# digitalcytometry/cytospace

Hardware: AMD Instinct MI355X
Metric: cell-to-spot assignments/sec on NxN synthetic cost; bit-exact vs lapjv (higher is better)
Workload: dtype f32

## Files before the change

cytospace_amd/csrc/lap_wide.hip:

```cpp
#include "lap_dev.h"
#include "lap_wide.h"
#include <algorithm>
#include <atomic>
#include <chrono>
#include <mutex>
#include <thread>
#include <vector>

namespace cyto {

#define WIDE_FIELDS(P, S)                                                                                                  \
    S(int, n) S(int64_t, ld) P(const float, cost) P(const int32_t, rowmap) P(float, v) P(float, u) P(float, cassign)          \
    P(unsigned long long, label) P(unsigned long long, bid) P(int32_t, rowsol) P(int32_t, colsol) P(int32_t, matches)          \
    P(int32_t, freerows) P(int32_t, act0) P(int32_t, act1) P(int32_t, touched) P(int32_t, slot_j) P(float, slot_p)            \
    P(float, slot_c) P(uint32_t, cache_col) P(float, cache_val) P(char, misc) S(long long, max_rounds)                     \
    P(const int32_t, same_prev) P(int32_t, seg_sync) S(int, aug_seg) S(int, aug_waste) S(int, arr_waste) S(int, seg_quorum)   \
    P(char, sc) S(int, par_groups) P(char, par) P(char, scx) P(float, cache_red) P(const int32_t, inv_off) P(const unsigned long long, inv_ent)
#define WIDE_F_PTR(T, name) T *name;
#define WIDE_F_VAL(T, name) T name;
struct WideArgs { WIDE_FIELDS(WIDE_F_PTR, WIDE_F_VAL) };

constexpr size_t WIDE_SC_BYTES = 2048;

namespace {
// ... 978 lines not shown
    int numfree = 0;
    for (int i0 = 0; i0 < n; i0 += WT) {
        const int i = i0 + tid;
        const bool fr = i < n && ld_sc1(a.rowsol + i) < 0;
        const uint64_t m = __ballot(fr);
        if (lane == 0) s.wcnt[w] = __popcll(m);
        __syncthreads();
        int pre = 0, tot = 0;
#pragma unroll
        for (int k = 0; k < WNW; k++) { const int c = s.wcnt[k]; if (k < w) pre += c; tot += c; }
        if (fr) a.freerows[numfree + pre + __popcll(m & lanemask_lt())] = i;
        numfree += tot;
        __syncthreads();
    }
    if (tid == 0) {
        long long *ctr = lap_status(a.misc)->counters;
        long long *wc = lap_status(a.misc)->wide;
        ctr[C_ARR] = bids; ctr[C_FREE_CR] = free_cr; ctr[C_FREE_A1] = numfree; ctr[C_FREE_A2] = numfree;
        wc[WC_ROUNDS] = round; wc[WC_BIDS] = bids; wc[WC_RETIRED] = s.retired; wc[WC_ACTIVE_LEFT] = left;
        wc[WC_FREE_ARR] = numfree; wc[WC_DENSE_ARR] = s.dense;
        lap_status(a.misc)->numfree = numfree;
        long long *tmr = lap_status(a.misc)->timers;
        tmr[WT_LIST_ROUNDS] = n_list; tmr[WT_LIST_TICKS] += t_list; tmr[WT_CHAIN_ROUNDS] = n_chain; tmr[WT_CHAIN_TICKS] += t_chain;
        tmr[WT_DEALS] = n_deal; tmr[WT_ARR_TAIL_TICKS] = wall_clock64() - t_tail0;
        h->started = 1; h->round = round; h->bids = bids; h->retired = s.retired; h->dense = s.dense; h->cnt[cur] = paused ? na : 0;
        h->cnt[cur ^ 1] = 0; h->free_cr = free_cr; h->done = paused ? 0 : 1; h->launches += 1; h->list_rounds = n_list;
#ifndef CYTO_WIDE_PROF
        tmr[WT_ARR_LAUNCHES] = h->launches;
#endif
        if (a.seg_sync) a.seg_sync[1 + blockIdx.x] = (paused ? 1 : 0) | ((!paused && s.dense <= n / 64) ? 2 : 0);
    }
}

struct ClaimCtl { int changed, blocked, rounds, pad_; };
__device__ __forceinline__ int *cl_claim(const WideArgs &a) { return reinterpret_cast<int *>(a.scx); }
__device__ __forceinline__ unsigned long long *cl_mask(const WideArgs &a) { return reinterpret_cast<unsigned long long *>(a.scx + sc_np(a.n) * 8); }
__device__ __forceinline__ int2 *cl_state(const WideArgs &a) { return reinterpret_cast<int2 *>(a.scx + sc_np(a.n) * 16); }
__device__ __forceinline__ ClaimCtl *cl_ctl(const WideArgs &a) { return reinterpret_cast<ClaimCtl *>(a.scx + sc_np(a.n) * 24); }
__device__ __forceinline__ int *cl_rem(const WideArgs &a) { return reinterpret_cast<int *>(a.scx + sc_np(a.n) * 32); }
constexpr int AP = 2;

size_t wide_aug_lds_bytes(int n, bool vlds, bool clds) {
    const size_t nblk = ((size_t)n + 63) / 64, nw32 = ((size_t)n + 31) / 32, npad = ((size_t)n + 3) & ~(size_t)3;
    return ((nblk * 8 + 3 * nw32 * 4 + npad * ((vlds ? 4 : 0) + (clds ? 2 : 0)) + 15) / 16) * 16;
}
bool wide_aug_vlds(int n) { return n <= 65534 && wide_aug_lds_bytes(n, true, true) + 4096 <= (size_t)LDS_DYNAMIC_MAX; }
bool wide_aug_clds(int n) { return n <= 65534 && wide_aug_lds_bytes(n, false, true) + 4096 <= (size_t)LDS_DYNAMIC_MAX; }

struct AugShared {
    unsigned long long T;
    int ntouch, any[3], npk[3], fail, anydense, rootdense, doroot, f, err;
    int waste, stop;
    int nhop;
    int conflict;
    int scans;
    int st_row[64], st_col[64];
    float st_val[64];
};
static_assert(WNW * AP <= 32, "the queue of a round's full-row relaxations: two halves of the 64-entry staging arrays");

struct ParCtl {
    unsigned int bar_arrive, bar_gen;
    int P[2], nplog[2], nolog[2];
    int err, pad_;
    long long c_relax, c_hops, c_proc, c_dense, c_rounds, c_verify, c_batches, c_discarded;
};
static_assert(sizeof(ParCtl) <= 256, "control block");
constexpr int PAR_GMAX = 64;
static size_t wide_par_state_bytes(int n, int G) {
    const size_t np = ((size_t)n + 63) & ~(size_t)63;
    return 256 + (size_t)G * np * 8 + (size_t)G * np * 4 + (size_t)G * np * 8 + np * 4 + np * 8 + np * 8;
}
__device__ __forceinline__ void par_barrier(ParCtl *c, int G, unsigned &gen) {
    __syncthreads();
    if (threadIdx.x == 0) {
        __builtin_amdgcn_fence(__ATOMIC_RELEASE, "agent");
        asm volatile("s_waitcnt vmcnt(0)" ::: "memory");
        const unsigned arrived = atomicAdd(&c->bar_arrive, 1u) + 1u;
        if (arrived == (gen + 1u) * (unsigned)G) st_sc1(&c->bar_gen, gen + 1u);
        else {
            long long spins = 0;
            while (ld_sc1(&c->bar_gen) <= gen) {
                __builtin_amdgcn_s_sleep(2);
                if (++spins > (1ll << 26)) { atomicExch(&c->err, 2); break; }
            }
        }
        __builtin_amdgcn_fence(__ATOMIC_ACQUIRE, "agent");
    }
    gen++;
    __syncthreads();
}

#ifndef CYTO_COOP_MIN_N
#define CYTO_COOP_MIN_N 16384
#endif
constexpr int COOP_MIN_N = CYTO_COOP_MIN_N;
template <bool VLDS>
__device__ __forceinline__ void coop_dense_rows(AugShared *sp, int nd, const float *__restrict__ cost, const int32_t *__restrict__ rowmap, int64_t ld,
                                             int n, int w, int lane, unsigned long long *lbl, int32_t *tch, uint32_t *dirty,
                                             unsigned long long *bmin, const uint32_t *asg, const float *s_v, const float *v) {
    AugShared &s = *sp;
    const int nq = (n + 3) >> 2, per = (nq + WNW - 1) / WNW, q_lo = w * per, q_hi = min(nq, q_lo + per);
    for (int e = 0; e < nd; e++) {
        const int oiq = uni(s.st_row[e]), pjq = uni(s.st_row[32 + e]);
        const uint32_t dord = (uint32_t)uni(s.st_col[e]), kq = (uint32_t)uni(s.st_col[32 + e]);
        const float h = uni(s.st_val[e]);
        const float *__restrict__ row = cost + wrow_off(rowmap, oiq, ld);
        wave_row_sweep_q(row, q_lo, q_hi, n, lane, [&](int c, float x) {
            const float vc = VLDS ? s_v[c] : ld_sc1(v + c);
            const unsigned long long lv = edge_lv(f2ord((x - vc) - h), dord, kq);
            const unsigned long long key = lkey(lv, (uint32_t)oiq);
            if (c == pjq || lv > lv_of(s.T) || !(key < ld_sc1(lbl + c))) return;
            const unsigned long long old = atomicMin(lbl + c, key);
            if (key < old) {
                if (old == ~0ull) tch[atomicAdd(&s.ntouch, 1)] = c;
                if (lv_of(old) > lv) {
                    const unsigned long long ck = lkey(lv, (uint32_t)c);
                    if ((asg[c >> 5] >> (c & 31)) & 1u) { atomicOr(&dirty[c >> 5], 1u << (c & 31)); atomicMin(&bmin[c >> 6], ck); }
                    else atomicMin(&s.T, ck);
                }
            }
        });
    }
    __syncthreads();
}

typedef __attribute__((address_space(1))) float gf32_t;
typedef __attribute__((address_space(1))) const int32_t gci32_t;
typedef __attribute__((address_space(1))) const unsigned long long gcu64_t;
__device__ __noinline__ void embed_repair(gf32_t *cache_red, gci32_t *inv_off, gcu64_t *inv_ent, uint64_t m, int k, float nv) {
    constexpr int U = 8;
    const int lane = threadIdx.x & 63;
    m = uni((unsigned long long)m);
    const bool mine = (m >> lane) & 1;
    const int e0 = mine ? inv_off[k] : 0, e1 = mine ? inv_off[k + 1] : 0;
    while (m) {
        int b[U], e[U]; float x[U]; unsigned long long t[U];
#pragma unroll
        for (int u = 0; u < U; u++) {
            const int l = m ? __ffsll((unsigned long long)m) - 1 : 0;
            b[u] = m ? __builtin_amdgcn_readlane(e0, l) : 0;
            e[u] = m ? __builtin_amdgcn_readlane(e1, l) : 0;
            x[u] = __uint_as_float((uint32_t)__builtin_amdgcn_readlane((int)__float_as_uint(nv), l));
            m &= m - 1;
        }
#pragma unroll
        for (int u = 0; u < U; u++) t[u] = b[u] + lane < e[u] ? inv_ent[b[u] + lane] : 0ull;
#pragma unroll
        for (int u = 0; u < U; u++) if (b[u] + lane < e[u]) cache_red[(uint32_t)t[u]] = __uint_as_float((uint32_t)(t[u] >> 32)) - x[u];
#pragma unroll
        for (int u = 0; u < U; u++)
            for (int p = b[u] + 64 + lane; p < e[u]; p += 64) { const unsigned long long y = inv_ent[p]; cache_red[(uint32_t)y] = __uint_as_float((uint32_t)(y >> 32)) - x[u]; }
    }
}

template <bool VLDS, bool CLDS, bool PAR, bool EMB = false>
__global__ __launch_bounds__(WT) void wide_aug(const WideArgs *__restrict__ batch) {
    static_assert(!EMB || (PAR && !VLDS), "the embedded form: several searches at once, prices in global memory");
    extern __shared__ __align__(16) unsigned char w_smem[];
    __shared__ AugShared s;
    const int pstride = PAR ? (int)(gridDim.x / (unsigned)load_wide_args(batch, 0).par_groups) : 1;
    if (PAR && (blockIdx.x % pstride)) return;
    const int g = PAR ? uni((int)(blockIdx.x / pstride)) : 0;
    const WideArgs a = load_wide_args(batch, PAR ? 0 : blockIdx.x);
    const int n = a.n, tid = threadIdx.x, lane = tid & 63, w = uni((int)(threadIdx.x >> 6));
    const int nblk = (n + 63) / 64, nw32 = (n + 31) / 32;
    const int G = PAR ? a.par_groups : 1;
    const size_t np_ = ((size_t)n + 63) & ~(size_t)63;
    ParCtl *pc = reinterpret_cast<ParCtl *>(a.par);
    unsigned long long *lbl = PAR ? reinterpret_cast<unsigned long long *>(a.par + 256) + (size_t)g * np_ : a.label;
    int32_t *tch = PAR ? reinterpret_cast<int32_t *>(a.par + 256 + (size_t)G * np_ * 8) + (size_t)g * np_ : a.touched;
    int32_t *hop_i = PAR ? reinterpret_cast<int32_t *>(a.par + 256 + (size_t)G * np_ * 12) + (size_t)g * 2 * np_ : a.act0;
    int32_t *hop_j = PAR ? hop_i + np_ : a.act1;
    uint32_t *claim = reinterpret_cast<uint32_t *>(a.par + 256 + (size_t)G * np_ * 20);
    int32_t *plog_col = reinterpret_cast<int32_t *>(claim + np_);
    float *plog_val = reinterpret_cast<float *>(plog_col + np_);
    int32_t *olog_col = reinterpret_cast<int32_t *>(plog_val + np_);
    int32_t *olog_own = olog_col + np_;
    unsigned pgen = 0;
    unsigned long long *bmin = reinterpret_cast<unsigned long long *>(w_smem);
    uint32_t *dirty = reinterpret_cast<uint32_t *>(bmin + nblk);
    uint32_t *asg = dirty + nw32;
    uint32_t *dense = asg + nw32;
    float *s_v = reinterpret_cast<float *>(dense + nw32);
    uint16_t *s_cs = reinterpret_cast<uint16_t *>(s_v + (VLDS ? ((n + 3) & ~3) : 0));
    const int numfree = lap_status(a.misc)->numfree;
    for (int b = tid; b < nblk; b += WT) bmin[b] = ~0ull;
    for (int q = tid; q < nw32; q += WT) { dirty[q] = 0; dense[q] = 0; }
    for (int c0 = 0; c0 < nw32 * 32; c0 += WT) {
        const int c = c0 + tid;
        const uint64_t m = __ballot(c < n && a.colsol[c] >= 0);
        if (lane == 0 && (c >> 5) < nw32) { asg[c >> 5] = (uint32_t)m; if ((c >> 5) + 1 < nw32) asg[(c >> 5) + 1] = (uint32_t)(m >> 32); }
    }
    if (CLDS)
        for (int j = tid; j < n; j += WT) {
            if (VLDS) s_v[j] = a.v[j];
            const int o = a.colsol[j]; s_cs[j] = o < 0 ? (uint16_t)0xFFFFu : (uint16_t)o;
        }
    const int f0 = PAR ? 0 : lap_status(a.misc)->wide_done;
    if (!PAR) {
        long long *wc = lap_status(a.misc)->wide;
        if (wc[WC_AUG_LAUNCHES] > 0 && f0 >= numfree) {
            if (tid == 0 && a.seg_sync) a.seg_sync[1 + blockIdx.x] = 0;
            return;
        }
    }
    if (tid == 0) { s.waste = 0; s.stop = 0; }
    if (tid == 0) { s.T = ~0ull; s.ntouch = 0; s.any[0] = 0; s.any[1] = 0; s.any[2] = 0; s.npk[0] = 0; s.npk[1] = 0; s.npk[2] = 0; s.fail = 0; s.anydense = 0; s.rootdense = 0; s.doroot = 0; s.f = f0; s.err = 0; s.scans = 0; }
    __syncthreads();
    auto getv = [&](int j) -> float { return VLDS ? s_v[j] : ld_sc1(a.v + j); };
    auto getcs = [&](int j) -> int {
        if (CLDS) { const uint16_t x = s_cs[j]; return x == 0xFFFFu ? -1 : (int)x; }
        return ld_sc1(a.colsol + j);
    };
    auto is_asg = [&](int c) -> bool { return (asg[c >> 5] >> (c & 31)) & 1u; };

    long long c_relax = 0, c_hops = 0, c_rounds = 0, c_proc = 0, c_trivial = 0, c_dense = 0, c_verify = 0;
    long long t_rounds = 0, t_verify = 0, t_finish = 0, t_triv = 0, t_mark = wall_clock64();

#define AUG_LAP(acc) { const long long now_ = wall_clock64(); acc += now_ - t_mark; t_mark = now_; }

    auto offer = [&](int col, unsigned long long lv, int row) -> unsigned long long {
        return atomicMin(lbl + col, lkey(lv, (uint32_t)row));
    };
    auto after_offer = [&](int col, unsigned long long lv, int row, unsigned long long old) {
        const unsigned long long key = lkey(lv, (uint32_t)row);
        if (key < old) {
            if (old == ~0ull) tch[atomicAdd(&s.ntouch, 1)] = col;
            if (lv_of(old) > lv) {
                const unsigned long long ck = lkey(lv, (uint32_t)col);
                if (is_asg(col)) { atomicOr(&dirty[col >> 5], 1u << (col & 31)); atomicMin(&bmin[col >> 6], ck); }
                else atomicMin(&s.T, ck);
            }
        }
    };
    auto relax_to = [&](int col, unsigned long long lv, int row) { after_offer(col, lv, row, offer(col, lv, row)); };

    int f = f0;
    int ph = 0;
    int rb[AP];
#pragma unroll
    for (int q = 0; q < AP; q++) rb[q] = -1;
    int seg_done = 0;
    int wact = 4;
    bool announced = false;
    int fbase = 0, batchno = 1, perr = 0;
    long long c_batches = 0, c_discarded = 0;
    for (;;) {
        if (!PAR && w == 0) {
            auto flush_one_edge = [&](int cnt) {
                if (lane < cnt) {
                    const int r = s.st_row[lane], cc = s.st_col[lane];
                    a.rowsol[r] = cc; a.colsol[cc] = r; a.cassign[cc] = s.st_val[lane];
                }
            };
            const int *remp = (a.same_prev && a.scx) ? cl_rem(a) : nullptr;
            int nst = 0;
            int p0, l0, r0, p1, l1, r1, p2, l2, r2, p3, l3v, r3v;
            uint32_t col0, col1, col2; float val0, val1, val2, vv0, vv1;
            auto start = [&](int ff) {
                auto len_of = [&](int pp) -> int { return pp < numfree ? (remp ? uni(remp[pp]) : 1) : 1; };
                auto row_at = [&](int pp) -> int { return pp < numfree ? uni(a.freerows[pp]) : -1; };
                p0 = ff; l0 = len_of(p0); r0 = row_at(p0);
                p1 = p0 + l0; l1 = len_of(p1); r1 = row_at(p1);
                p2 = p1 + l1; l2 = len_of(p2); r2 = row_at(p2);
                p3 = p2 + l2; l3v = p3 < numfree ? (remp ? remp[p3] : 1) : 1; r3v = p3 < numfree ? a.freerows[p3] : -1;
                col0 = COLSENT; col1 = COLSENT; col2 = COLSENT; val0 = 0.0f; val1 = 0.0f; val2 = 0.0f;
                if (r0 >= 0) { col0 = a.cache_col[(int64_t)r0 * KC + lane]; val0 = a.cache_val[(int64_t)r0 * KC + lane]; }
                if (r1 >= 0) { col1 = a.cache_col[(int64_t)r1 * KC + lane]; val1 = a.cache_val[(int64_t)r1 * KC + lane]; }
                if (r2 >= 0) { col2 = a.cache_col[(int64_t)r2 * KC + lane]; val2 = a.cache_val[(int64_t)r2 * KC + lane]; }
                vv0 = (r0 >= 0 && lane < KCU && col0 != COLSENT) ? getv((int)col0) : 0.0f;
                vv1 = (r1 >= 0 && lane < KCU && col1 != COLSENT) ? getv((int)col1) : 0.0f;
            };
// ... 227 lines not shown
                ph = (ph + 1) % 3;
                c_rounds++;
                wact = np > 6 ? WNW : 4;
                nd = npd >> 16;
                if (!any || nd) break;
            }
            if (nd) {
                coop_dense_rows<VLDS>(&s, nd, a.cost, a.rowmap, a.ld, n, w, lane, lbl, tch, dirty, bmin, asg, s_v, a.v);
                continue;
            }
            AUG_LAP(t_rounds)
            const unsigned long long Tk = s.T;
            const uint32_t Dord = (uint32_t)(Tk >> 32);
            const float D = Tk == ~0ull ? INFINITY : ord2f(Dord);
            const int nt = s.ntouch;
            for (int q = tid; q < nt; q += WT) {
                const int k = ld_sc1(tch + q);
                const unsigned long long lbk = ld_sc1(lbl + k);
                const uint32_t dord = (uint32_t)(lbk >> 32);
                if (lv_of(lbk) < lv_of(Tk) && is_asg(k)) {
                    const int i = getcs(k);
                    if (!((dense[i >> 5] >> (i & 31)) & 1u)) {
                        const float h = (ld_sc1(a.cassign + k) - getv(k)) - ord2f(dord);
                        const float bound = a.cache_val[(int64_t)i * KC + KCU] - h;
                        if (!(bound > D)) {
                            atomicOr(&dense[i >> 5], 1u << (i & 31));
                            atomicOr(&dirty[k >> 5], 1u << (k & 31));
                            atomicMin(&bmin[k >> 6], lkey(lv_of(lbk), (uint32_t)k));
                            atomicAdd(&s.fail, 1);
                        }
                    }
                }
            }
            if (tid == 0 && !s.rootdense && !(ftau > D)) { s.rootdense = 1; s.doroot = 1; atomicAdd(&s.fail, 1); }
            c_verify++;
            __syncthreads();
            const int fail = s.fail;
            if (s.doroot)
                for (int c = tid; c < n; c += WT) {
                    const unsigned long long lv = (unsigned long long)f2ord(frow[c] - getv(c)) << 12;
                    if (lv <= lv_of(s.T) && (lkey(lv, (uint32_t)fr) < ld_sc1(lbl + c))) relax_to(c, lv, fr);
                }
            __syncthreads();
            if (tid == 0) { if (fail) s.anydense = 1; s.fail = 0; s.doroot = 0; }
            __syncthreads();
            AUG_LAP(t_verify)
            if (!fail) break;
        }

        }

        const unsigned long long Tk = active ? s.T : ~0ull;
        if (!PAR && Tk == ~0ull) { if (tid == 0) s.err = 1; __syncthreads(); break; }
        const uint32_t Dord = (uint32_t)(Tk >> 32);
        const float D = ord2f(Dord);
        const int sink = (int)lid_of(Tk);
        const int nt = active ? s.ntouch : 0;
        bool commit = true;
        int Pb = G;
        const int par = batchno & 1;
        if (PAR) {
            const bool have = Tk != ~0ull;
            if (active && !have && tid == 0) atomicExch(&pc->err, 1);
            const uint32_t key = ((uint32_t)batchno << 8) | (uint32_t)(255 - g);
            if (have) {
                for (int q = tid; q < nt; q += WT) {
                    const int k = ld_sc1(tch + q);
                    if (lv_of(ld_sc1(lbl + k)) < lv_of(Tk) && is_asg(k)) atomicMax(claim + k, key);
                }
                if (tid == 0) atomicMax(claim + sink, key);
            }
            if (tid == 0) s.conflict = 0;
            par_barrier(pc, G, pgen);
            if (have) {
                int c = 0;
                for (int q = tid; q < nt; q += WT) {
                    const int k = ld_sc1(tch + q);
                    if (lv_of(ld_sc1(lbl + k)) < lv_of(Tk) && is_asg(k) && ld_sc1(claim + k) != key) c = 1;
                }
                if (tid == 0 && ld_sc1(claim + sink) != key) c = 1;
                if (c) s.conflict = 1;
            }
            __syncthreads();
            if (tid == 0 && active && (s.conflict || !have)) atomicMin(&pc->P[par], g);
            par_barrier(pc, G, pgen);
            Pb = uni(ld_sc1(&pc->P[par]));
            Pb = Pb < G ? Pb : G;
            if (g == 0 && tid == 0) { st_sc1(&pc->P[par ^ 1], PAR_GMAX + 1); st_sc1(&pc->nplog[par ^ 1], 0); st_sc1(&pc->nolog[par ^ 1], 0); }
            commit = active && have && g < Pb;
            if (active && !commit) c_discarded++;
        }
        if (commit) {
            int myscans = 0;
            for (int q = tid; q < nt; q += WT) {
                const int k = ld_sc1(tch + q);
                const uint32_t dord = (uint32_t)(ld_sc1(lbl + k) >> 32);
                if (dord < Dord && is_asg(k)) {
                    const float vk = getv(k);
                    const float nv = (vk + ord2f(dord)) - D;
                    if (nv < vk) {
                        a.v[k] = nv; if (VLDS) s_v[k] = nv;
                        if (PAR) { const int e = atomicAdd(&pc->nplog[par], 1); plog_col[e] = k; plog_val[e] = nv; }
                    }
                    myscans++;
                }
            }
            if (myscans) atomicAdd(&s.scans, myscans);
            if (tid == 0) {
                int j = sink, nh = 0;
                for (;;) {
                    const int i = (int)lid_of(ld_sc1(lbl + j));
                    const int jn = ld_sc1(a.rowsol + i);
                    a.colsol[j] = i; a.rowsol[i] = j;
                    st_sc1(hop_i + nh, (int32_t)i); st_sc1(hop_j + nh, (int32_t)j); nh++;
                    if (CLDS) s_cs[j] = (uint16_t)i;
                    c_hops++;
                    if (i == fr) break;
                    j = jn;
                }
                s.nhop = nh;
                atomicOr(&asg[sink >> 5], 1u << (sink & 31));
            }
            __syncthreads();
            for (int q = tid; q < s.nhop; q += WT) {
                const int i = ld_sc1(hop_i + q), j = ld_sc1(hop_j + q);
                a.cassign[j] = a.cost[wrow_off(a.rowmap, i, a.ld) + j];
                if (PAR) { const int e = atomicAdd(&pc->nolog[par], 1); olog_col[e] = j; olog_own[e] = i; }
            }
        }
        for (int q = tid; q < nt; q += WT) {
            const int k = ld_sc1(tch + q);
            lbl[k] = ~0ull;
            atomicAnd(&dirty[k >> 5], ~(1u << (k & 31)));
            bmin[k >> 6] = ~0ull;
        }
        if (s.anydense) for (int q = tid; q < nw32; q += WT) dense[q] = 0;
        __syncthreads();
        if (tid == 0) { if (commit) c_relax += s.scans; s.scans = 0; s.T = ~0ull; s.ntouch = 0; s.anydense = 0; s.rootdense = 0; s.f = f + 1; }
        f++;
        __syncthreads();
        if (PAR) {
            par_barrier(pc, G, pgen);
            perr = uni(ld_sc1(&pc->err));
            const int npl = uni(ld_sc1(&pc->nplog[par])), nol = uni(ld_sc1(&pc->nolog[par]));
            if (VLDS) for (int e = tid; e < npl; e += WT) s_v[ld_sc1(plog_col + e)] = ld_sc1(plog_val + e);
            for (int e = tid; e < nol; e += WT) {
                const int col = ld_sc1(olog_col + e);
                if (CLDS) s_cs[col] = (uint16_t)ld_sc1(olog_own + e);
                atomicOr(&asg[col >> 5], 1u << (col & 31));
            }
            __syncthreads();
            const int left = numfree - fbase;
            fbase += Pb < left ? Pb : left;
            if (Pb < 1) perr = 1;
            if (EMB) {
                for (int e0 = (g * WNW + w) * 8; e0 < npl; e0 += G * WNW * 8) {
                    const bool have_e = lane < 8 && e0 + lane < npl;
                    const int k = have_e ? ld_sc1(plog_col + e0 + lane) : 0;
                    const float nv = have_e ? ld_sc1(plog_val + e0 + lane) : 0.0f;
                    embed_repair((gf32_t *)a.cache_red, (gci32_t *)a.inv_off, (gcu64_t *)a.inv_ent, __ballot(have_e), k, nv);
                }
                par_barrier(pc, G, pgen);
            }
            batchno++; c_batches++;
        }
        AUG_LAP(t_finish)
    }

    __syncthreads();
    __shared__ double s_tot[WNW];
    __shared__ long long s_wc[WNW][4];
    if (lane == 0) { s_wc[w][0] = c_proc; s_wc[w][1] = c_dense; s_wc[w][2] = c_trivial; s_wc[w][3] = (w == 0) ? c_hops : 0; }
    __syncthreads();
    long long proc = 0, dn = 0, triv = 0, hops0 = 0;
    for (int k = 0; k < WNW; k++) { proc += s_wc[k][0]; dn += s_wc[k][1]; triv += s_wc[k][2]; hops0 += s_wc[k][3]; }
    if (PAR) {
        if (tid == 0) {
            atomicAdd(reinterpret_cast<unsigned long long *>(&pc->c_relax), (unsigned long long)c_relax);
            atomicAdd(reinterpret_cast<unsigned long long *>(&pc->c_hops), (unsigned long long)hops0);
            atomicAdd(reinterpret_cast<unsigned long long *>(&pc->c_proc), (unsigned long long)proc);
            atomicAdd(reinterpret_cast<unsigned long long *>(&pc->c_dense), (unsigned long long)dn);
            atomicAdd(reinterpret_cast<unsigned long long *>(&pc->c_discarded), (unsigned long long)c_discarded);
            if (g == 0) { pc->c_rounds = c_rounds; pc->c_verify = c_verify; pc->c_batches = c_batches; }
        }
        par_barrier(pc, G, pgen);
        if (g != 0) return;
        c_relax = (long long)ld_sc1(reinterpret_cast<unsigned long long *>(&pc->c_relax));
        hops0 = (long long)ld_sc1(reinterpret_cast<unsigned long long *>(&pc->c_hops));
        proc = (long long)ld_sc1(reinterpret_cast<unsigned long long *>(&pc->c_proc));
        dn = (long long)ld_sc1(reinterpret_cast<unsigned long long *>(&pc->c_dense));
        f = perr || ld_sc1(&pc->err) ? f : numfree;
    }
    double tot = 0.0;
    for (int i = tid; i < n; i += WT) {
        const int j = ld_sc1(a.rowsol + i);
        if (j >= 0) {
            const float cij = ld_sc1(a.cassign + j);
            a.u[i] = cij - ld_sc1(a.v + j);
            tot += (double)cij;
        }
    }
#pragma unroll
    for (int off = 32; off > 0; off >>= 1) tot += __shfl_xor(tot, off);
    if (lane == 0) s_tot[w] = tot;
    __syncthreads();
    if (tid == 0) {
        double t = 0.0;
        for (int k = 0; k < WNW; k++) t += s_tot[k];
        const bool err = s.err || (PAR && (perr || ld_sc1(&pc->err)));
        LapStatus *st = lap_status(a.misc);
        st->total = t;
        long long *ctr = st->counters, *wc = st->wide;
        ctr[C_AUG_INIT] = numfree; ctr[C_AUG_RELAX] += c_relax; ctr[C_AUGS] = numfree; ctr[C_HOPS] += hops0;
        wc[WC_DENSE_AUG] += dn; wc[WC_AUG_LAUNCHES] += 1; wc[WC_AUG_ROUNDS] += c_rounds; wc[WC_AUG_PROCESSED] += proc; wc[WC_TRIVIAL] += triv; wc[WC_VERIFY_PASSES] += c_verify;
        if (err) st->status = 1;
        st->wide_done = err ? numfree : f;
// ... 428 lines not shown
        const int xcd_cus = std::max(1, pl.cache.cus / 8);
        const bool dup_rows = n >= 2 && (long long)j.ngroups * 5 < (long long)n * 4;
        int parg = nl != 1 ? 0 : (pl.par > 0 ? pl.par : (pl.par < 0 || dup_rows || n < 2048 ? 0 : 16));
        parg = std::min(std::min(parg, WIDE_PAR_GMAX), xcd_cus);
        if (parg == 1) parg = 0;
        if (parg > 1) {
            if (g_par_busy[device_slot].exchange(1) != 0) parg = 0;
            else par_slot.p = &g_par_busy[device_slot];
        }
        const size_t parb = parg > 0 ? wide_par_state_bytes(n, parg) : 0;
        const size_t sc_off = ((2 * nT + 255) / 256) * 256;
        const size_t par_off = sc_off + WIDE_SC_BYTES;
        const size_t scx_off = ((par_off + parb + 255) / 256) * 256;
        bool vlds_k, clds_k;
        wide_aug_lds_choice(n, vlds_k, clds_k);
        const bool emb_cand = parg > 1 && !vlds_k && n <= (1 << 25) && embed_knob != 0;
        const size_t emb_off = ((scx_off + wide_sc_ext_bytes(n) + 255) / 256) * 256;
        if ((rc = j.state->alloc(emb_cand ? emb_off + wide_embed_bytes(n) : scx_off + wide_sc_ext_bytes(n), stream))) return rc;
        WideArgs &wa = h_wa[(size_t)k];
        wa.cache_red = nullptr; wa.inv_off = nullptr; wa.inv_ent = nullptr;
        if (emb_cand) {
            char *eb = j.state->as<char>() + emb_off;
            wa.cache_red = reinterpret_cast<float *>(eb);
            wa.inv_off = reinterpret_cast<int32_t *>(eb + emb_a256((size_t)n * KC * 4));
            wa.inv_ent = reinterpret_cast<unsigned long long *>(eb + emb_off_ent(n));
        }
        wa.n = n; wa.ld = j.ld; wa.cost = j.cost; wa.rowmap = j.rowmap;
        wa.v = j.fws; wa.u = j.fws + n; wa.cassign = j.fws + 3 * (int64_t)n;
        wa.label = reinterpret_cast<unsigned long long *>(j.fws + 4 * (int64_t)n);
        wa.rowsol = j.iws; wa.colsol = j.iws + n; wa.matches = j.iws + 2 * (int64_t)n; wa.freerows = j.iws + 3 * (int64_t)n;
        wa.act0 = j.iws + 4 * (int64_t)n; wa.act1 = j.iws + 5 * (int64_t)n; wa.touched = j.iws + 6 * (int64_t)n;
        wa.slot_j = j.iws + 7 * (int64_t)n;
        wa.bid = reinterpret_cast<unsigned long long *>(j.iws + 8 * (int64_t)n);
        wa.slot_p = j.state->as<float>(); wa.slot_c = wa.slot_p + n;
        wa.cache_col = j.cache_col; wa.cache_val = j.cache_val; wa.misc = j.misc;
        wa.max_rounds = pl.rounds;
        wa.aug_seg = pl.rebuild;
        wa.aug_waste = (int)std::min<long long>(1 << 30, std::max<long long>(16, (2000000ll + (long long)nl * n * n / 100) / n));
        wa.arr_waste = std::max(8, wa.aug_waste / 3);
        if (CYTO_KNOB("CYTO_ARR_WASTE").set) wa.arr_waste = std::max(1, CYTO_KNOB("CYTO_ARR_WASTE").value);
        wa.seg_quorum = nl > 1 ? std::max(1, nl / 4) : 0;
        wa.seg_sync = nullptr;
        wa.same_prev = j.same;
        wa.sc = j.state->as<char>() + sc_off;
        CYTO_HIP(hipMemsetAsync(wa.sc, 0, WIDE_SC_BYTES, stream));
        wa.scx = j.state->as<char>() + scx_off;
        CYTO_HIP(hipMemsetAsync(wa.scx, 0, wide_sc_ext_bytes(n), stream));
        CYTO_HIP(hipMemsetAsync(wa.scx, 0xFF, wide_sc_ones_bytes(n), stream));
        wa.par_groups = parg; wa.par = nullptr;
        if (parg > 0) {
            const size_t np_ = ((size_t)n + 63) & ~(size_t)63;
            wa.par = j.state->as<char>() + par_off;
            CYTO_HIP(hipMemsetAsync(wa.par, 0, 256, stream));
            const int p_init[2] = {WIDE_PAR_GMAX + 1, WIDE_PAR_GMAX + 1};
            CYTO_HIP(hipMemcpyAsync(wa.par + 8, p_init, sizeof p_init, hipMemcpyHostToDevice, stream));
            CYTO_HIP(hipMemsetAsync(wa.par + 256, 0xFF, (size_t)parg * np_ * 8, stream));
            CYTO_HIP(hipMemsetAsync(wa.par + 256 + (size_t)parg * np_ * 20, 0, np_ * 4, stream));
            CYTO_HIP(hipStreamSynchronize(stream));
        }
        CYTO_HIP(hipMemcpyAsync(wa.cassign, wa.v, nT, hipMemcpyDeviceToDevice, stream));
        CYTO_HIP(hipMemsetAsync(wa.label, 0xFF, 2 * nT, stream));
        CYTO_HIP(hipMemsetAsync(wa.bid, 0xFF, 2 * nT, stream));
    }
    DevBuf d_wa, d_sync;
    if ((rc = d_wa.alloc(sizeof(WideArgs) * nl, stream)) || (rc = d_sync.alloc(sizeof(int32_t) * ((size_t)nl + 1), stream))) return rc;
    for (WideArgs &wa : h_wa) wa.seg_sync = d_sync.as<int32_t>();
    CYTO_HIP(hipMemcpyAsync(d_wa.p, h_wa.data(), sizeof(WideArgs) * nl, hipMemcpyHostToDevice, stream));
    if ((rc = wide_launch_rt(d_wa.as<WideArgs>(), nl, n, stream))) return rc;
    std::vector<int32_t> h_sync((size_t)nl + 1, 1);
    std::vector<int32_t> caches_fresh((size_t)nl, 0);
    using BuildFn = decltype(build_caches_of);
    auto rebuild_tramp = +[](void *ctx, const int32_t *flags) -> int { return (*static_cast<BuildFn *>(ctx))(flags); };
    for (int pass = 0;; pass++) {
        if (pass && (rc = build_caches_of(h_sync.data() + 1))) return rc;
        CYTO_HIP(hipMemsetAsync(d_sync.p, 0, sizeof(int32_t), stream));
        if ((rc = wide_launch_arr(d_wa.as<WideArgs>(), nl, n, stream, pl.wipe, pass > 0, d_sync.as<int32_t>(), rebuild_tramp, &build_caches_of,
                                  nl == 1 ? &h_wa[0] : nullptr))) return rc;
        if (h_wa[0].aug_seg != 0) break;
        CYTO_HIP(hipMemcpyAsync(h_sync.data(), d_sync.p, sizeof(int32_t) * ((size_t)nl + 1), hipMemcpyDeviceToHost, stream));
        CYTO_HIP(hipStreamSynchronize(stream));
        bool done = true;
        for (int k = 0; k < nl; k++) { done = done && (h_sync[(size_t)k + 1] & 1) == 0; caches_fresh[(size_t)k] = (h_sync[(size_t)k + 1] & 2) != 0; h_sync[(size_t)k + 1] &= 1; }
        if (done) break;
    }
    const int parg = h_wa[0].par_groups;
    for (int pass = 0;; pass++) {
        if (pass == 0) {
            std::vector<int32_t> need((size_t)nl);
            for (int k = 0; k < nl; k++) need[(size_t)k] = caches_fresh[(size_t)k] ? 0 : 1;
            if ((rc = build_caches_of(need.data()))) return rc;
        } else if ((rc = build_caches_of(h_sync.data() + 1))) return rc;
        if (pass == 0) CYTO_HIP(hipEventRecord(ev_arr_done, stream));
        if (pass == 0 && parg == 0) {
            bool dup = false;
            for (int k = 0; k < nl; k++) dup = dup || h_wa[(size_t)k].same_prev != nullptr;
            if (dup && (rc = wide_launch_claims(d_wa.as<WideArgs>(), nl, n, stream, d_sync.as<int32_t>()))) return rc;
        }
        bool embed = false;
        if (parg > 0 && h_wa[0].cache_red) {
            if ((rc = wide_build_embedded(h_wa[0], n, stream))) return rc;
            embed = embed_knob >= 2;
            if (!embed) {
                int32_t longest = 0;
                CYTO_HIP(hipMemcpyAsync(&longest, emb_counts(h_wa[0], n) + n, sizeof longest, hipMemcpyDeviceToHost, stream));
                CYTO_HIP(hipStreamSynchronize(stream));
                embed = longest <= EMB_GATE;
            }
        }
        CYTO_HIP(hipMemsetAsync(d_sync.p, 0, sizeof(int32_t), stream));
        if ((rc = wide_launch_aug(d_wa.as<WideArgs>(), nl, n, stream, parg, embed))) return rc;
        if (embed) g_embedded_solves.fetch_add(1);
        if (parg > 0) { CYTO_HIP(hipStreamSynchronize(stream)); break; }
        CYTO_HIP(hipMemcpyAsync(h_sync.data(), d_sync.p, sizeof(int32_t) * ((size_t)nl + 1), hipMemcpyDeviceToHost, stream));
        CYTO_HIP(hipStreamSynchronize(stream));
        bool done = true;
        for (int k = 0; k < nl; k++) done = done && h_sync[(size_t)k + 1] == 0;
        if (done) break;
    }
    return CYTO_OK;
}

void wide_info(cyto_lap_info *info, const LapStatus &h) {
    const long long *wc = h.wide, *tm = h.timers;
    info->wide = 1;
    info->aug_handover = -1;
    info->wide_rounds = wc[WC_ROUNDS]; info->wide_retired = wc[WC_RETIRED]; info->wide_dense_arr = wc[WC_DENSE_ARR];
    info->wide_dense_aug = wc[WC_DENSE_AUG]; info->wide_aug_rounds = wc[WC_AUG_ROUNDS]; info->wide_aug_settled = wc[WC_AUG_PROCESSED];
    info->wide_trivial = wc[WC_TRIVIAL]; info->wide_verify_passes = wc[WC_VERIFY_PASSES]; info->wide_aug_launches = wc[WC_AUG_LAUNCHES];
    info->wide_list_rounds = tm[WT_LIST_ROUNDS]; info->wide_chain_rounds = tm[WT_CHAIN_ROUNDS];
    info->wide_ms_list = tm[WT_LIST_TICKS] * 1e-5; info->wide_ms_chain = tm[WT_CHAIN_TICKS] * 1e-5;
    info->wide_ms_aug_rounds = tm[WT_AUG_ROUNDS_TICKS] * 1e-5; info->wide_ms_aug_verify = tm[WT_AUG_VERIFY_TICKS] * 1e-5;
    info->wide_ms_aug_finish = tm[WT_AUG_FINISH_TICKS] * 1e-5; info->wide_ms_aug_trivial = tm[WT_AUG_TRIVIAL_TICKS] * 1e-5;
    info->wide_arr_launches = tm[WT_ARR_LAUNCHES]; info->wide_scaled = tm[WT_SCALED]; info->wide_phases = tm[WT_PHASES];
    info->wide_par_batches = tm[WT_PAR_BATCHES]; info->wide_par_discarded = tm[WT_PAR_DISCARDED];
}

}

extern "C" long long cyto_wide_embedded_solves(void) { return cyto::g_embedded_solves.load(); }
```

Before: 1.337 million.

## Restructure parallel augment finish: single-barrier claim, parallel price update, link-based path walk

Moves the end-of-search commit into a separate noinline routine. The claim phase now detects conflicts from the atomicMax return value instead of a second barrier-and-verify pass, which removes one grid-wide barrier per batch. Settled columns are logged into a per-group set list that a later batched price update reads. The augmenting-path walk runs in wave 0, using precomputed row links with 4-hop jumps, while the other waves update prices concurrently. Hop writes are batched, log appends use wave-aggregated atomics, and a host stream sync plus an H2D copy are dropped. The cost is extra global state and more complex, riskier conflict logic.

```diff
diff --git a/cytospace_amd/csrc/lap_wide.hip b/cytospace_amd/csrc/lap_wide.hip
--- a/cytospace_amd/csrc/lap_wide.hip
+++ b/cytospace_amd/csrc/lap_wide.hip
@@ -1054,7 +1054,7 @@
     int ntouch, any[3], npk[3], fail, anydense, rootdense, doroot, f, err;
     int waste, stop;
     int nhop;
-    int conflict;
+    int nset;
     int scans;
     int st_row[64], st_col[64];
     float st_val[64];
@@ -1069,10 +1069,48 @@
 };
 static_assert(sizeof(ParCtl) <= 256, "control block");
 constexpr int PAR_GMAX = 64;
+#ifdef CYTO_AUG_FIN_SPLIT
+constexpr int FS_MAXB = 2048, FS_G = 16, FS_NP = 14;
+enum { FS_CLAIM, FS_WAIT1, FS_CHECK, FS_WAIT2, FS_UPDATE, FS_WALK, FS_COST, FS_RESET, FS_WAIT3, FS_REPAIR, FS_NTOUCH, FS_SETTLED, FS_HOPS, FS_ARRIVE };
+__device__ long long g_fs[FS_MAXB][FS_G][FS_NP];
+#define FS_OK (PAR && batchno - 1 < FS_MAXB && g < FS_G)
+#define FS_BEGIN() { if (PAR && tid == 0) { fs_mark = wall_clock64(); if (FS_OK) g_fs[batchno - 1][g][FS_ARRIVE] = fs_mark; } }
+#define FS_LAP(part) { if (PAR) { __syncthreads(); if (tid == 0) { const long long fsn_ = wall_clock64(); if (FS_OK) g_fs[batchno - 1][g][part] = fsn_ - fs_mark; fs_mark = fsn_; } } }
+#define FS_SET(part, val) { if (tid == 0 && FS_OK) g_fs[batchno - 1][g][part] = (val); }
+#define FS_COUNT() atomicAdd(&s.st_col[63], 1)
+#else
+#define FS_BEGIN()
+#define FS_LAP(part)
+#define FS_SET(part, val)
+#define FS_COUNT()
+#endif
 static size_t wide_par_state_bytes(int n, int G) {
     const size_t np = ((size_t)n + 63) & ~(size_t)63;
-    return 256 + (size_t)G * np * 8 + (size_t)G * np * 4 + (size_t)G * np * 8 + np * 4 + np * 8 + np * 8;
-}
+    return 256 + (size_t)G * np * 8 + (size_t)G * np * 4 + (size_t)G * np * 8 + np * 4 + np * 8 + np * 8 + (size_t)G * np * 8 + (size_t)G * np * 8 +
+           (size_t)G * np * 32;
+}
+struct SearchView {
+    unsigned long long *lbl, *setl, *link, *link4;
+    int32_t *tch, *hop_i, *hop_j, *plog_col, *olog_col, *olog_own;
+    uint32_t *claim;
+    float *plog_val;
+    __device__ __forceinline__ SearchView(const WideArgs &a, bool par, int g) {
+        const int G = par ? a.par_groups : 1;
+        const size_t np_ = ((size_t)a.n + 63) & ~(size_t)63;
+        lbl = par ? reinterpret_cast<unsigned long long *>(a.par + 256) + (size_t)g * np_ : a.label;
+        tch = par ? reinterpret_cast<int32_t *>(a.par + 256 + (size_t)G * np_ * 8) + (size_t)g * np_ : a.touched;
+        hop_i = par ? reinterpret_cast<int32_t *>(a.par + 256 + (size_t)G * np_ * 12) + (size_t)g * 2 * np_ : a.act0;
+        hop_j = par ? hop_i + np_ : a.act1;
+        claim = reinterpret_cast<uint32_t *>(a.par + 256 + (size_t)G * np_ * 20);
+        plog_col = reinterpret_cast<int32_t *>(claim + np_);
+        plog_val = reinterpret_cast<float *>(plog_col + np_);
+        olog_col = reinterpret_cast<int32_t *>(plog_val + np_);
+        olog_own = olog_col + np_;
+        setl = reinterpret_cast<unsigned long long *>(olog_own + np_) + (size_t)g * np_;
+        link = reinterpret_cast<unsigned long long *>(olog_own + np_) + ((size_t)G + (size_t)g) * np_;
+        link4 = reinterpret_cast<unsigned long long *>(olog_own + np_) + (2 * (size_t)G + 4 * (size_t)g) * np_;
+    }
+};
 __device__ __forceinline__ void par_barrier(ParCtl *c, int G, unsigned &gen) {
     __syncthreads();
     if (threadIdx.x == 0) {
@@ -1156,6 +1194,264 @@
     }
 }
 
+typedef __attribute__((address_space(3))) struct AugShared lds_aug_t;
+typedef __attribute__((address_space(3))) unsigned long long lds_u64_t;
+#ifndef CYTO_WALK_LINKS
+#define CYTO_WALK_LINKS 1
+#endif
+#ifndef CYTO_WALK_HOP4
+#define CYTO_WALK_HOP4 1
+#endif
+template <bool VLDS, bool CLDS, bool PAR>
+__device__ __noinline__ unsigned long long search_end(const WideArgs *__restrict__ batch, lds_aug_t *sp, lds_u64_t *smem, int g_, int fr_, int batchno_,
+                                                      unsigned pgen_, int active_) {
+    constexpr bool LINKS = PAR && CYTO_WALK_LINKS;
+    AugShared &s = *(AugShared *)sp;
+    const int g = uni(g_), fr = uni(fr_), batchno = uni(batchno_);
+    unsigned pgen = uni(pgen_);
+    const bool active = uni(active_) != 0;
+    const WideArgs a = load_wide_args(batch, PAR ? 0 : blockIdx.x);
+    const int n = a.n, tid = threadIdx.x, lane = tid & 63, w = uni((int)(threadIdx.x >> 6));
+    const int nblk = (n + 63) / 64, nw32 = (n + 31) / 32;
+    const int G = PAR ? a.par_groups : 1;
+    ParCtl *pc = reinterpret_cast<ParCtl *>(a.par);
+    const SearchView sv(a, PAR, g);
+    unsigned long long *lbl = sv.lbl, *setl = sv.setl, *link = sv.link;
+    int32_t *tch = sv.tch, *hop_i = sv.hop_i, *hop_j = sv.hop_j;
+    unsigned long long *bmin = (unsigned long long *)smem;
+    uint32_t *dirty = reinterpret_cast<uint32_t *>(bmin + nblk);
+    uint32_t *asg = dirty + nw32;
+    uint32_t *dense = asg + nw32;
+    float *s_v = reinterpret_cast<float *>(dense + nw32);
+    uint16_t *s_cs = reinterpret_cast<uint16_t *>(s_v + (VLDS ? ((n + 3) & ~3) : 0));
+    auto getv = [&](int j) -> float { return VLDS ? s_v[j] : ld_sc1(a.v + j); };
+    auto is_asg = [&](int c) -> bool { return (asg[c >> 5] >> (c & 31)) & 1u; };
+#ifdef CYTO_AUG_FIN_SPLIT
+    long long fs_mark = 0;
+#endif
+    const unsigned long long Tk = active ? uni((unsigned long long)s.T) : ~0ull;
+    const uint32_t Dord = (uint32_t)(Tk >> 32);
+    const float D = ord2f(Dord);
+    const int sink = (int)lid_of(Tk);
+    const int nt = active ? uni(s.ntouch) : 0;
+    const int par = batchno & 1;
+    bool commit = true;
+    int Pb = G;
+    FS_BEGIN()
+    if (PAR) {
+        const bool have = Tk != ~0ull;
+        if (active && !have && tid == 0) { atomicExch(&pc->err, 1); atomicMin(&pc->P[par], g); }
+        const uint32_t key = ((uint32_t)batchno << 8) | (uint32_t)(255 - g);
+        auto flag = [&](uint32_t old) {
+            if ((old >> 8) == (uint32_t)batchno && old != key) {
+                const int go = 255 - (int)(old & 255u);
+                atomicMin(&pc->P[par], g > go ? g : go);
+            }
+        };
+        if (have) {
+            constexpr int CU_ = 4;
+            for (int q0 = 0; q0 < nt; q0 += CU_ * WT) {
+                int k[CU_], pre[CU_], cnt = 0;
+                unsigned long long lb[CU_];
+                uint64_t m[CU_];
+                bool st[CU_];
+#pragma unroll
+                for (int t = 0; t < CU_; t++) { const int q = q0 + t * WT + tid; k[t] = q < nt ? ld_sc1(tch + q) : -1; }
+#pragma unroll
+                for (int t = 0; t < CU_; t++) lb[t] = k[t] >= 0 ? ld_sc1(lbl + k[t]) : ~0ull;
+#pragma unroll
+                for (int t = 0; t < CU_; t++) {
+                    st[t] = k[t] >= 0 && lv_of(lb[t]) < lv_of(Tk) && is_asg(k[t]);
+                    m[t] = __ballot(st[t]); pre[t] = cnt; cnt += __popcll(m[t]);
+                }
+                if (cnt == 0) continue;
+                int rs[CU_];
+#pragma unroll
+                for (int t = 0; t < CU_; t++) rs[t] = LINKS && st[t] ? ld_sc1(a.rowsol + (int)lid_of(lb[t])) : -1;
+                uint32_t old[CU_];
+#pragma unroll
+                for (int t = 0; t < CU_; t++) old[t] = st[t] ? atomicMax(sv.claim + k[t], key) : 0u;
+                int base = 0;
+                if (lane == 0) base = atomicAdd(&s.nset, cnt);
+                base = uni(base);
+#pragma unroll
+                for (int t = 0; t < CU_; t++)
+                    if (st[t]) {
+                        setl[base + pre[t] + __popcll(m[t] & lanemask_lt())] = (lb[t] >> 32 << 32) | (uint32_t)k[t];
+                        if (LINKS) link[k[t]] = ((unsigned long long)(uint32_t)rs[t] << 32) | lid_of(lb[t]);
+                        flag(old[t]);
+                        FS_COUNT();
+                    }
+            }
+            if (tid == 0) flag(atomicMax(sv.claim + sink, key));
+        }
+        FS_LAP(FS_CLAIM)
+        par_barrier(pc, G, pgen);
+        FS_LAP(FS_WAIT1)
+        Pb = uni(ld_sc1(&pc->P[par]));
+        Pb = Pb < G ? Pb : G;
+        if (g == 0 && tid == 0) { st_sc1(&pc->P[par ^ 1], PAR_GMAX + 1); st_sc1(&pc->nplog[par ^ 1], 0); st_sc1(&pc->nolog[par ^ 1], 0); }
+        commit = active && have && g < Pb;
+    }
+    int nhop = 0;
+    if (commit) {
+        const int nset = PAR ? uni(s.nset) : 0;
+        const bool hop4 = LINKS && CYTO_WALK_HOP4 && nset >= 32;
+        if (hop4) {
+            const unsigned long long END = 0xFFFFFFFF00000000ull | (uint32_t)fr;
+            for (int q = tid; q < nset; q += WT) {
+                const int k = (int)(uint32_t)ld_sc1(setl + q);
+                unsigned long long *dst = sv.link4 + 4 * (size_t)k;
+                unsigned long long e[4];
+                e[0] = ld_sc1(link + k);
+#pragma unroll
+                for (int d = 1; d < 4; d++) e[d] = (int)(uint32_t)e[d - 1] != fr ? ld_sc1(link + (uint32_t)(e[d - 1] >> 32)) : END;
+#pragma unroll
+                for (int d = 0; d < 4; d++) dst[d] = e[d];
+            }
+            __syncthreads();
+        }
+        if (w == 0) {
+#ifdef CYTO_AUG_FIN_SPLIT
+            const long long fs_w0 = wall_clock64();
+#endif
+            int nh = 0, mi = 0, mj = 0;
+            auto rec = [&](int ri, int rj) {
+                if (lane == (nh & 63)) { mi = ri; mj = rj; }
+                nh++;
+                if ((nh & 63) == 0 && nh <= n) { st_sc1(hop_i + nh - 64 + lane, (int32_t)mi); st_sc1(hop_j + nh - 64 + lane, (int32_t)mj); }
+            };
+            int j = sink;
+            int i = uni((int)lid_of(ld_sc1(lbl + sink)));
+            rec(i, j);
+            if (i != fr) {
+                j = uni(ld_sc1(a.rowsol + i));
+                while (nh < n) {
+                    if (hop4) {
+                        unsigned long long e[4];
+#pragma unroll
+                        for (int t = 0; t < 4; t++) e[t] = ld_sc1(sv.link4 + 4 * (size_t)j + t);
+                        bool done = false;
+#pragma unroll
+                        for (int t = 0; t < 4; t++)
+                            if (!done) {
+                                const unsigned long long lk = uni(e[t]);
+                                i = (int)(uint32_t)lk; rec(i, j);
+                                if (i == fr) done = true; else j = (int)(uint32_t)(lk >> 32);
+                            }
+                        if (done) break;
+                    } else if (LINKS) {
+                        const unsigned long long lk = uni(ld_sc1(link + j));
+                        i = (int)(uint32_t)lk; rec(i, j);
+                        if (i == fr) break;
+                        j = (int)(uint32_t)(lk >> 32);
+                    } else {
+                        i = uni((int)lid_of(ld_sc1(lbl + j))); rec(i, j);
+                        if (i == fr) break;
+                        j = uni(ld_sc1(a.rowsol + i));
+                    }
+                }
+            }
+            if (nh > n) nh = n;
+            if (lane < (nh & 63)) { st_sc1(hop_i + (nh & ~63) + lane, (int32_t)mi); st_sc1(hop_j + (nh & ~63) + lane, (int32_t)mj); }
+            if (lane == 0) s.nhop = nh;
+            if (lane == 0 && i != fr) { if (PAR) atomicExch(&pc->err, 1); else s.err = 1; }
+#ifdef CYTO_AUG_FIN_SPLIT
+            if (lane == 0 && FS_OK) g_fs[batchno - 1][g][FS_WALK] = wall_clock64() - fs_w0;
+#endif
+        } else {
+            constexpr int UT = WT - 64;
+            const int ne = PAR ? uni(s.nset) : nt;
+            int myscans = 0;
+            for (int q0 = 0; q0 < ne; q0 += 4 * UT) {
+                int k[4], pre[4], cnt = 0;
+                uint32_t dord[4];
+                float vk[4], nv[4];
+                uint64_t m[4];
+                bool up[4];
+                if (PAR) {
+#pragma unroll
+                    for (int t = 0; t < 4; t++) {
+                        const int q = q0 + t * UT + tid - 64;
+                        const unsigned long long e = q < ne ? ld_sc1(setl + q) : ~0ull;
+                        k[t] = (int)(uint32_t)e; dord[t] = (uint32_t)(e >> 32);
+                        up[t] = q < ne && dord[t] < Dord;
+                    }
+                } else {
+#pragma unroll
+                    for (int t = 0; t < 4; t++) { const int q = q0 + t * UT + tid - 64; k[t] = q < ne ? ld_sc1(tch + q) : -1; }
+#pragma unroll
+                    for (int t = 0; t < 4; t++) {
+                        dord[t] = k[t] >= 0 ? (uint32_t)(ld_sc1(lbl + k[t]) >> 32) : 0xFFFFFFFFu;
+                        up[t] = k[t] >= 0 && dord[t] < Dord && is_asg(k[t]);
+                    }
+                }
+#pragma unroll
+                for (int t = 0; t < 4; t++) vk[t] = up[t] ? getv(k[t]) : 0.0f;
+#pragma unroll
+                for (int t = 0; t < 4; t++) {
+                    nv[t] = (vk[t] + ord2f(dord[t])) - D;
+                    myscans += up[t] ? 1 : 0;
+                    up[t] = up[t] && nv[t] < vk[t];
+                    if (up[t]) { a.v[k[t]] = nv[t]; if (VLDS) s_v[k[t]] = nv[t]; }
+                    if (PAR) { m[t] = __ballot(up[t]); pre[t] = cnt; cnt += __popcll(m[t]); }
+                }
+                if (PAR && cnt) {
+                    int base = 0;
+                    if (lane == 0) base = atomicAdd(&pc->nplog[par], cnt);
+                    base = uni(base);
+#pragma unroll
+                    for (int t = 0; t < 4; t++)
+                        if (up[t]) { const int e = base + pre[t] + __popcll(m[t] & lanemask_lt()); sv.plog_col[e] = k[t]; sv.plog_val[e] = nv[t]; }
+                }
+            }
+            if (myscans) atomicAdd(&s.scans, myscans);
+        }
+        __syncthreads();
+        FS_LAP(FS_UPDATE)
+        nhop = uni(s.nhop);
+        for (int q0 = 0; q0 < nhop; q0 += WT) {
+            const int q = q0 + tid;
+            const bool hv = q < nhop;
+            const int i = hv ? ld_sc1(hop_i + q) : 0, j = hv ? ld_sc1(hop_j + q) : 0;
+            if (hv) {
+                a.colsol[j] = i; a.rowsol[i] = j;
+                if (CLDS) s_cs[j] = (uint16_t)i;
+                a.cassign[j] = a.cost[wrow_off(a.rowmap, i, a.ld) + j];
+            }
+            if (PAR) {
+                const uint64_t m = __ballot(hv);
+                if (m) {
+                    int base = 0;
+                    if (lane == 0) base = atomicAdd(&pc->nolog[par], __popcll(m));
+                    base = uni(base);
+                    if (hv) { const int e = base + __popcll(m & lanemask_lt()); sv.olog_col[e] = j; sv.olog_own[e] = i; }
+                }
+            }
+        }
+        if (tid == 0) atomicOr(&asg[sink >> 5], 1u << (sink & 31));
+        FS_SET(FS_HOPS, nhop)
+        FS_LAP(FS_COST)
+    }
+    for (int q0 = 0; q0 < nt; q0 += 4 * WT) {
+        int k[4];
+#pragma unroll
+        for (int t = 0; t < 4; t++) { const int q = q0 + t * WT + tid; k[t] = q < nt ? ld_sc1(tch + q) : -1; }
+#pragma unroll
+        for (int t = 0; t < 4; t++)
+            if (k[t] >= 0) {
+                lbl[k[t]] = ~0ull;
+                atomicAnd(&dirty[k[t] >> 5], ~(1u << (k[t] & 31)));
+                bmin[k[t] >> 6] = ~0ull;
+            }
+    }
+    if (s.anydense) for (int q = tid; q < nw32; q += WT) dense[q] = 0;
+    __syncthreads();
+    FS_SET(FS_NTOUCH, nt)
+    FS_LAP(FS_RESET)
+    return (unsigned long long)(uint32_t)nhop | ((unsigned long long)(uint32_t)Pb << 32) | ((unsigned long long)(commit ? 1 : 0) << 48);
+}
+
 template <bool VLDS, bool CLDS, bool PAR, bool EMB = false>
 __global__ __launch_bounds__(WT) void wide_aug(const WideArgs *__restrict__ batch) {
     static_assert(!EMB || (PAR && !VLDS), "the embedded form: several searches at once, prices in global memory");
@@ -1168,17 +1464,11 @@
     const int n = a.n, tid = threadIdx.x, lane = tid & 63, w = uni((int)(threadIdx.x >> 6));
     const int nblk = (n + 63) / 64, nw32 = (n + 31) / 32;
     const int G = PAR ? a.par_groups : 1;
-    const size_t np_ = ((size_t)n + 63) & ~(size_t)63;
     ParCtl *pc = reinterpret_cast<ParCtl *>(a.par);
-    unsigned long long *lbl = PAR ? reinterpret_cast<unsigned long long *>(a.par + 256) + (size_t)g * np_ : a.label;
-    int32_t *tch = PAR ? reinterpret_cast<int32_t *>(a.par + 256 + (size_t)G * np_ * 8) + (size_t)g * np_ : a.touched;
-    int32_t *hop_i = PAR ? reinterpret_cast<int32_t *>(a.par + 256 + (size_t)G * np_ * 12) + (size_t)g * 2 * np_ : a.act0;
-    int32_t *hop_j = PAR ? hop_i + np_ : a.act1;
-    uint32_t *claim = reinterpret_cast<uint32_t *>(a.par + 256 + (size_t)G * np_ * 20);
-    int32_t *plog_col = reinterpret_cast<int32_t *>(claim + np_);
-    float *plog_val = reinterpret_cast<float *>(plog_col + np_);
-    int32_t *olog_col = reinterpret_cast<int32_t *>(plog_val + np_);
-    int32_t *olog_own = olog_col + np_;
+    const SearchView sv(a, PAR, g);
+    unsigned long long *lbl = sv.lbl;
+    int32_t *tch = sv.tch, *plog_col = sv.plog_col, *olog_col = sv.olog_col, *olog_own = sv.olog_own;
+    float *plog_val = sv.plog_val;
     unsigned pgen = 0;
     unsigned long long *bmin = reinterpret_cast<unsigned long long *>(w_smem);
     uint32_t *dirty = reinterpret_cast<uint32_t *>(bmin + nblk);
@@ -1208,7 +1498,7 @@
         }
     }
     if (tid == 0) { s.waste = 0; s.stop = 0; }
-    if (tid == 0) { s.T = ~0ull; s.ntouch = 0; s.any[0] = 0; s.any[1] = 0; s.any[2] = 0; s.npk[0] = 0; s.npk[1] = 0; s.npk[2] = 0; s.fail = 0; s.anydense = 0; s.rootdense = 0; s.doroot = 0; s.f = f0; s.err = 0; s.scans = 0; }
+    if (tid == 0) { s.T = ~0ull; s.ntouch = 0; s.any[0] = 0; s.any[1] = 0; s.any[2] = 0; s.npk[0] = 0; s.npk[1] = 0; s.npk[2] = 0; s.fail = 0; s.anydense = 0; s.rootdense = 0; s.doroot = 0; s.f = f0; s.err = 0; s.scans = 0; s.nset = 0; }
     __syncthreads();
     auto getv = [&](int j) -> float { return VLDS ? s_v[j] : ld_sc1(a.v + j); };
     auto getcs = [&](int j) -> int {
@@ -1221,6 +1511,11 @@
     long long t_rounds = 0, t_verify = 0, t_finish = 0, t_triv = 0, t_mark = wall_clock64();
 
 #define AUG_LAP(acc) { const long long now_ = wall_clock64(); acc += now_ - t_mark; t_mark = now_; }
+#ifdef CYTO_AUG_FIN_SPLIT
+    long long fs_mark = 0;
+    if (tid == 0) s.st_col[63] = 0;
+    __syncthreads();
+#endif
 
     auto offer = [&](int col, unsigned long long lv, int row) -> unsigned long long {
         return atomicMin(lbl + col, lkey(lv, (uint32_t)row));
@@ -1554,93 +1849,19 @@
 
         const unsigned long long Tk = active ? s.T : ~0ull;
         if (!PAR && Tk == ~0ull) { if (tid == 0) s.err = 1; __syncthreads(); break; }
-        const uint32_t Dord = (uint32_t)(Tk >> 32);
-        const float D = ord2f(Dord);
-        const int sink = (int)lid_of(Tk);
-        const int nt = active ? s.ntouch : 0;
-        bool commit = true;
-        int Pb = G;
+        const unsigned long long er = uni(search_end<VLDS, CLDS, PAR>(batch, (lds_aug_t *)&s, (lds_u64_t *)w_smem, g, fr, batchno, pgen, active ? 1 : 0));
+        if (PAR) pgen++;
+        const bool commit = (er >> 48) & 1;
+        const int Pb = (int)((er >> 32) & 0xFFFFu);
         const int par = batchno & 1;
-        if (PAR) {
-            const bool have = Tk != ~0ull;
-            if (active && !have && tid == 0) atomicExch(&pc->err, 1);
-            const uint32_t key = ((uint32_t)batchno << 8) | (uint32_t)(255 - g);
-            if (have) {
-                for (int q = tid; q < nt; q += WT) {
-                    const int k = ld_sc1(tch + q);
-                    if (lv_of(ld_sc1(lbl + k)) < lv_of(Tk) && is_asg(k)) atomicMax(claim + k, key);
-                }
-                if (tid == 0) atomicMax(claim + sink, key);
-            }
-            if (tid == 0) s.conflict = 0;
-            par_barrier(pc, G, pgen);
-            if (have) {
-                int c = 0;
-                for (int q = tid; q < nt; q += WT) {
-                    const int k = ld_sc1(tch + q);
-                    if (lv_of(ld_sc1(lbl + k)) < lv_of(Tk) && is_asg(k) && ld_sc1(claim + k) != key) c = 1;
-                }
-                if (tid == 0 && ld_sc1(claim + sink) != key) c = 1;
-                if (c) s.conflict = 1;
-            }
-            __syncthreads();
-            if (tid == 0 && active && (s.conflict || !have)) atomicMin(&pc->P[par], g);
-            par_barrier(pc, G, pgen);
-            Pb = uni(ld_sc1(&pc->P[par]));
-            Pb = Pb < G ? Pb : G;
-            if (g == 0 && tid == 0) { st_sc1(&pc->P[par ^ 1], PAR_GMAX + 1); st_sc1(&pc->nplog[par ^ 1], 0); st_sc1(&pc->nolog[par ^ 1], 0); }
-            commit = active && have && g < Pb;
-            if (active && !commit) c_discarded++;
-        }
-        if (commit) {
-            int myscans = 0;
-            for (int q = tid; q < nt; q += WT) {
-                const int k = ld_sc1(tch + q);
-                const uint32_t dord = (uint32_t)(ld_sc1(lbl + k) >> 32);
-                if (dord < Dord && is_asg(k)) {
-                    const float vk = getv(k);
-                    const float nv = (vk + ord2f(dord)) - D;
-                    if (nv < vk) {
-                        a.v[k] = nv; if (VLDS) s_v[k] = nv;
-                        if (PAR) { const int e = atomicAdd(&pc->nplog[par], 1); plog_col[e] = k; plog_val[e] = nv; }
-                    }
-                    myscans++;
-                }
-            }
-            if (myscans) atomicAdd(&s.scans, myscans);
-            if (tid == 0) {
-                int j = sink, nh = 0;
-                for (;;) {
-                    const int i = (int)lid_of(ld_sc1(lbl + j));
-                    const int jn = ld_sc1(a.rowsol + i);
-                    a.colsol[j] = i; a.rowsol[i] = j;
-                    st_sc1(hop_i + nh, (int32_t)i); st_sc1(hop_j + nh, (int32_t)j); nh++;
-                    if (CLDS) s_cs[j] = (uint16_t)i;
-                    c_hops++;
-                    if (i == fr) break;
-                    j = jn;
-                }
-                s.nhop = nh;
-                atomicOr(&asg[sink >> 5], 1u << (sink & 31));
-            }
-            __syncthreads();
-            for (int q = tid; q < s.nhop; q += WT) {
-                const int i = ld_sc1(hop_i + q), j = ld_sc1(hop_j + q);
-                a.cassign[j] = a.cost[wrow_off(a.rowmap, i, a.ld) + j];
-                if (PAR) { const int e = atomicAdd(&pc->nolog[par], 1); olog_col[e] = j; olog_own[e] = i; }
-            }
-        }
-        for (int q = tid; q < nt; q += WT) {
-            const int k = ld_sc1(tch + q);
-            lbl[k] = ~0ull;
-            atomicAnd(&dirty[k >> 5], ~(1u << (k & 31)));
-            bmin[k >> 6] = ~0ull;
-        }
-        if (s.anydense) for (int q = tid; q < nw32; q += WT) dense[q] = 0;
-        __syncthreads();
-        if (tid == 0) { if (commit) c_relax += s.scans; s.scans = 0; s.T = ~0ull; s.ntouch = 0; s.anydense = 0; s.rootdense = 0; s.f = f + 1; }
+        c_hops += (long long)(uint32_t)er;
+        if (PAR && active && !commit) c_discarded++;
+        if (tid == 0) { if (commit) c_relax += s.scans; s.scans = 0; s.T = ~0ull; s.ntouch = 0; s.nset = 0; s.anydense = 0; s.rootdense = 0; s.f = f + 1; }
         f++;
         __syncthreads();
+#ifdef CYTO_AUG_FIN_SPLIT
+        if (PAR && tid == 0) fs_mark = wall_clock64();
+#endif
         if (PAR) {
             par_barrier(pc, G, pgen);
             perr = uni(ld_sc1(&pc->err));
@@ -1652,6 +1873,7 @@
                 atomicOr(&asg[col >> 5], 1u << (col & 31));
             }
             __syncthreads();
+            FS_LAP(FS_WAIT3)
             const int left = numfree - fbase;
             fbase += Pb < left ? Pb : left;
             if (Pb < 1) perr = 1;
@@ -1664,6 +1886,11 @@
                 }
                 par_barrier(pc, G, pgen);
             }
+            FS_LAP(FS_REPAIR)
+#ifdef CYTO_AUG_FIN_SPLIT
+            FS_SET(FS_SETTLED, s.st_col[63])
+            if (tid == 0) s.st_col[63] = 0;
+#endif
             batchno++; c_batches++;
         }
         AUG_LAP(t_finish)
@@ -2198,11 +2425,9 @@
             const size_t np_ = ((size_t)n + 63) & ~(size_t)63;
             wa.par = j.state->as<char>() + par_off;
             CYTO_HIP(hipMemsetAsync(wa.par, 0, 256, stream));
-            const int p_init[2] = {WIDE_PAR_GMAX + 1, WIDE_PAR_GMAX + 1};
-            CYTO_HIP(hipMemcpyAsync(wa.par + 8, p_init, sizeof p_init, hipMemcpyHostToDevice, stream));
+            CYTO_HIP(hipMemsetD32Async(reinterpret_cast<hipDeviceptr_t>(wa.par + 8), WIDE_PAR_GMAX + 1, 2, stream));
             CYTO_HIP(hipMemsetAsync(wa.par + 256, 0xFF, (size_t)parg * np_ * 8, stream));
             CYTO_HIP(hipMemsetAsync(wa.par + 256 + (size_t)parg * np_ * 20, 0, np_ * 4, stream));
-            CYTO_HIP(hipStreamSynchronize(stream));
         }
         CYTO_HIP(hipMemcpyAsync(wa.cassign, wa.v, nT, hipMemcpyDeviceToDevice, stream));
         CYTO_HIP(hipMemsetAsync(wa.label, 0xFF, 2 * nT, stream));
@@ -2284,3 +2509,16 @@
 }
 
 extern "C" long long cyto_wide_embedded_solves(void) { return cyto::g_embedded_solves.load(); }
+
+#ifdef CYTO_AUG_FIN_SPLIT
+extern "C" int cyto_wide_fin_split(long long *out, int *max_batches, int *groups, int *parts) {
+    using namespace cyto;
+    *max_batches = FS_MAXB; *groups = FS_G; *parts = FS_NP;
+    if (!out) return 0;
+    if (hipDeviceSynchronize() != hipSuccess) return 5;
+    if (hipMemcpyFromSymbol(out, HIP_SYMBOL(g_fs), sizeof(long long) * FS_MAXB * FS_G * FS_NP) != hipSuccess) return 5;
+    void *p = nullptr;
+    if (hipGetSymbolAddress(&p, HIP_SYMBOL(g_fs)) != hipSuccess || hipMemset(p, 0, sizeof(long long) * FS_MAXB * FS_G * FS_NP) != hipSuccess) return 5;
+    return 0;
+}
+#endif
```

Result: faster. 1.364 million, median of 6 (+2.0%).
